# kxhit/SG_PR

Hardware: AMD Instinct MI355X
Metric: graph-pairs/sec (higher is better)
Workload: dtype f32 (2xf16-plane operands on the matrix cores, fp32 accumulate; fp32 vector math)

## Files before the change

sg_pr_amd/csrc/sgpr_score.hip:

```cpp
#include <math.h>

#include <string.h>

#include <type_traits>

#include "sgpr_internal.hpp"

namespace sgpr {

constexpr int F = kF3;
constexpr int T = kT;
constexpr int BN_ = kB;

__device__ __forceinline__ float ntn_neuron(const float* __restrict__ ntn_w, const float* __restrict__ ntn_wb,
                                            const float* __restrict__ bias, const float* __restrict__ e1,
                                            const float* __restrict__ e2, int lane) {
    const int t = lane & 15, q = lane >> 4;
    float v[8];
#pragma unroll
    for (int r = 0; r < 8; ++r) v[r] = 0.f;
    for (int i = 0; i < F; ++i) {
        const float a = e1[i];
        const float* wr = ntn_w + i * (F * T) + lane;
#pragma unroll
        for (int r = 0; r < 8; ++r) v[r] = fmaf(a, wr[64 * r], v[r]);
    }
    float s = 0.f;
#pragma unroll
    for (int r = 0; r < 8; ++r) s = fmaf(v[r], e2[q + 4 * r], s);
    for (int m = 0; m < 16; ++m) {
        const int mm = q * 16 + m;
        const float x = mm < F ? e1[mm] : e2[mm - F];
        s = fmaf(ntn_wb[t * 2 * F + mm], x, s);
    }
    s += __shfl_xor(s, 16);
    s += __shfl_xor(s, 32);
    return relu_keep_nan(s + bias[t]);
}

__global__ __launch_bounds__(256) void score_pairs_kernel(const DevWeights w, const float* __restrict__ p1,
                                                          const int32_t* __restrict__ i1,
                                                          const float* __restrict__ p2,
                                                          const int32_t* __restrict__ i2, int64_t P,
                                                          float* __restrict__ score) {
    const int lane = threadIdx.x & 63;
    const int64_t pair = (int64_t)blockIdx.x * 4 + (threadIdx.x >> 6);
    if (pair >= P) return;
    const int64_t r1 = i1 ? i1[pair] : pair;
    const int64_t r2 = i2 ? i2[pair] : pair;
    const int t = lane & 15;
    const float h = ntn_neuron(w.ntn_w, w.ntn_wb, w.ntn_bias, p1 + r1 * F, p2 + r2 * F, lane);
    float gacc = w.fc1_b[t];
    for (int tt = 0; tt < T; ++tt) gacc = fmaf(w.fc1_w[t * T + tt], __shfl(h, tt), gacc);
    float z = relu_keep_nan(gacc) * w.fc2_w[t];
    z += __shfl_xor(z, 1);
    z += __shfl_xor(z, 2);
    z += __shfl_xor(z, 4);
    z += __shfl_xor(z, 8);
    if (lane == 0) score[pair] = 1.f / (1.f + expf(-(z + w.fc2_b[0])));
}

__global__ __launch_bounds__(256) void ntn_kernel(const float* __restrict__ ntn_w, const float* __restrict__ ntn_wb,
                                                  const float* __restrict__ bias, const float* __restrict__ e1,
                                                  const float* __restrict__ e2, int64_t B, float* __restrict__ out) {
    const int lane = threadIdx.x & 63;
    const int64_t pair = (int64_t)blockIdx.x * 4 + (threadIdx.x >> 6);
    if (pair >= B) return;
    const float h = ntn_neuron(ntn_w, ntn_wb, bias, e1 + pair * F, e2 + pair * F, lane);
    if (lane < T) out[pair * T + lane] = h;
}

int launch_ntn(const float* w, const float* wb, const float* bias, const float* e1, const float* e2, int64_t B,
               float* out, hipStream_t stream) {
    if (B == 0) return SGPR_OK;
    const int64_t blocks = (B + 3) / 4;
    if (blocks > 0x7fffffffLL) {
        set_error("sgpr_ntn: too many pairs for one launch");
        return SGPR_E_INVALID;
    }
    hipLaunchKernelGGL(ntn_kernel, dim3((unsigned)blocks), dim3(256), 0, stream, w, wb, bias, e1, e2, B, out);
    hipError_t e = hipGetLastError();
    if (e != hipSuccess) return hip_fail(e, "ntn_kernel launch");
    return SGPR_OK;
}

int launch_score_pairs(const sgpr_handle* h, const float* p1, const int32_t* i1, const float* p2, const int32_t* i2,
                       int64_t P, float* score, hipStream_t stream) {
    if (P == 0) return SGPR_OK;
    const int64_t blocks = (P + 3) / 4;
    if (blocks > 0x7fffffffLL) {
        set_error("sgpr_score_pairs: too many pairs for one launch");
        return SGPR_E_INVALID;
    }
    hipLaunchKernelGGL(score_pairs_kernel, dim3((unsigned)blocks), dim3(256), 0, stream, h->w, p1, i1, p2, i2, P, score);
    hipError_t e = hipGetLastError();
    if (e != hipSuccess) return hip_fail(e, "score_pairs_kernel launch");
    return SGPR_OK;
}

constexpr int AP_RW = 4;
constexpr int AP_ROWS = 16;
constexpr int AP_SB = 64;
constexpr int AP_COLS = 256;
#ifndef SGPR_AP_OCC
#define SGPR_AP_OCC 4
#endif
constexpr int AP_MULTI_OCC = 3;
constexpr int AP_OCC = SGPR_AP_OCC;
#ifndef SGPR_AP_NI
#define SGPR_AP_NI 2
#endif
#ifndef SGPR_AP_CHAINS
#define SGPR_AP_CHAINS 1
#endif
#ifndef SGPR_AP_NT_STORE
#define SGPR_AP_NT_STORE 0
#endif
constexpr int AP_NI = SGPR_AP_NI;
constexpr float AP_F16_SAFE = 60000.f;

static inline int ap_prep_groups(int R, int M) {
    const int msb = (M + AP_SB - 1) / AP_SB * AP_SB;
    return ((R > msb ? R : msb) + 15) / 16;
}

size_t score_all_pairs_ws_bytes(int R, int M) {
    const size_t nsb = (size_t)(M + AP_SB - 1) / AP_SB;
    return (size_t)R * T * sizeof(float) + (size_t)2 * ap_prep_groups(R, M) * 4 * sizeof(float) +
           (size_t)R * 3 * 64 * 8 * sizeof(unsigned short) + nsb * 3 * 4 * 64 * 8 * sizeof(unsigned short);
}

struct ApOperands {
    float* ur;
    float* rng;
    unsigned short* Ab;
    unsigned short* Cb;
};
static ApOperands ap_operands(void* ws, int R, int nrng, int planes) {
    ApOperands o;
    o.ur = static_cast<float*>(ws);
    o.rng = o.ur + (size_t)R * T;
    o.Ab = reinterpret_cast<unsigned short*>(o.rng + (size_t)nrng * 4);
    o.Cb = o.Ab + (size_t)R * planes * 64 * 8;
    return o;
}

typedef float f32x4 __attribute__((ext_vector_type(4)));
typedef _Float16 f16x8 __attribute__((ext_vector_type(8)));
typedef _Float16 f16x2 __attribute__((ext_vector_type(2)));

__device__ __forceinline__ void split2_f16(float a, _Float16& h, _Float16& l) {
    h = (_Float16)a;
    l = (_Float16)(a - (float)h);
}

__device__ __forceinline__ void split3_bf16(float x, unsigned& hb, unsigned& mb, unsigned& lb) {
    hb = __float_as_uint(x);
    const float r1 = x - __uint_as_float(hb & 0xffff0000u);
    mb = __float_as_uint(r1);
    const float r2 = r1 - __uint_as_float(mb & 0xffff0000u);
    lb = __float_as_uint(r2);
}

__device__ __forceinline__ float range_max(float m, float x) { return fmaxf(m, x != x ? INFINITY : fabsf(x)); }

__device__ __forceinline__ float wave_max_f32(float v) {
    v = fmaxf(v, __shfl_xor(v, 1));
    v = fmaxf(v, __shfl_xor(v, 2));
    v = fmaxf(v, __shfl_xor(v, 4));
    v = fmaxf(v, __shfl_xor(v, 8));
    v = fmaxf(v, __shfl_xor(v, 16));
    return fmaxf(v, __shfl_xor(v, 32));
}

template <bool LIST, int NPL = 2>
__device__ __forceinline__ void ntn_prep_body(const DevWeights& w, const float* __restrict__ rows, int R,
                                              const float* __restrict__ cols, int M, unsigned short* __restrict__ Ab,
                                              float* __restrict__ ur, float* __restrict__ rng,
                                              unsigned short* __restrict__ Cb, const int block,
                                              const int32_t* __restrict__ row_ids = nullptr) {
    __shared__ float red[4][4];
    __shared__ __attribute__((aligned(16))) unsigned short stage[16 * NPL * 4 * 8 * 8];
    const int lane = threadIdx.x & 63, wave = threadIdx.x >> 6;
    const int l15 = lane & 15, lq = lane >> 4;
    const int g0 = (block >> 1) * 16, half = block & 1;
    float amax = 0.f, umax = 0.f, emax = 0.f, l1max = 0.f;
    if (g0 < R) {
        const int ga = min(g0 + l15, R - 1);
        const float* e = rows + (size_t)(LIST ? row_ids[ga] : ga) * F + 4 * lq;
        const float4 ea0 = *reinterpret_cast<const float4*>(e), ea1 = *reinterpret_cast<const float4*>(e + 16);
        float wv[4][8], wbv[4], l1r[4] = {0.f, 0.f, 0.f, 0.f};
#pragma unroll
        for (int q = 0; q < 4; ++q) {
            const int tile = half * 16 + wave * 4 + q;
            const int t = tile >> 1, j = (tile & 1) * 16 + l15;
            const float* wp = w.ntn_wt + ((size_t)(4 * lq) * T + t) * F + j;
#pragma unroll
            for (int s4 = 0; s4 < 4; ++s4) {
                wv[q][s4] = wp[s4 * T * F];
                wv[q][4 + s4] = wp[(16 + s4) * T * F];
            }
            wbv[q] = w.ntn_wb[t * 2 * F + F + j];
        }
#pragma unroll
        for (int q = 0; q < 4; ++q) {
            const int tile = half * 16 + wave * 4 + q;
            const int t = tile >> 1, j = (tile & 1) * 16 + l15;
            f32x4 acc = {0.f, 0.f, 0.f, 0.f};
            acc = __builtin_amdgcn_mfma_f32_16x16x4f32(ea0.x, wv[q][0], acc, 0, 0, 0);
            acc = __builtin_amdgcn_mfma_f32_16x16x4f32(ea0.y, wv[q][1], acc, 0, 0, 0);
            acc = __builtin_amdgcn_mfma_f32_16x16x4f32(ea0.z, wv[q][2], acc, 0, 0, 0);
            acc = __builtin_amdgcn_mfma_f32_16x16x4f32(ea0.w, wv[q][3], acc, 0, 0, 0);
            acc = __builtin_amdgcn_mfma_f32_16x16x4f32(ea1.x, wv[q][4], acc, 0, 0, 0);
            acc = __builtin_amdgcn_mfma_f32_16x16x4f32(ea1.y, wv[q][5], acc, 0, 0, 0);
            acc = __builtin_amdgcn_mfma_f32_16x16x4f32(ea1.z, wv[q][6], acc, 0, 0, 0);
            acc = __builtin_amdgcn_mfma_f32_16x16x4f32(ea1.w, wv[q][7], acc, 0, 0, 0);
            const float wbc = wbv[q];
            if ((q & 1) == 0) {
#pragma unroll
                for (int r = 0; r < 4; ++r) l1r[r] = 0.f;
            }
#pragma unroll
            for (int r = 0; r < 4; ++r) {
                const int g = g0 + 4 * lq + r;
                if (g < R) {
                    const float a = acc[r] + wbc;
                    amax = range_max(amax, a);
                    l1r[r] += fabsf(a);
                    unsigned short* dst = stage + (((4 * lq + r) * NPL * 4 + (j >> 3)) * 8 + (t & 7)) * 8 + (j & 7);
                    if constexpr (NPL == 3) {
                        unsigned hb, mb, lb;
                        split3_bf16(a, hb, mb, lb);
                        dst[0] = (unsigned short)(hb >> 16);
                        dst[4 * 8 * 8] = (unsigned short)(mb >> 16);
                        dst[2 * 4 * 8 * 8] = (unsigned short)(lb >> 16);
                    } else {
                        _Float16 h, l;
                        split2_f16(a, h, l);
                        dst[0] = __builtin_bit_cast(unsigned short, h);
                        dst[4 * 8 * 8] = __builtin_bit_cast(unsigned short, l);
                    }
                }
            }
            if (q & 1) {
#pragma unroll
                for (int r = 0; r < 4; ++r) {
                    float v = l1r[r];
                    v += __shfl_xor(v, 1);
                    v += __shfl_xor(v, 2);
                    v += __shfl_xor(v, 4);
                    v += __shfl_xor(v, 8);
                    l1max = fmaxf(l1max, v);
                }
            }
        }
    }
    if (g0 < R) {
        __syncthreads();
        for (int u = threadIdx.x; u < 16 * NPL * 4 * 8; u += 256) {
            const int tl = u & 7, jb = (u >> 3) & 3, pl = (u >> 5) % NPL, gi = (u >> 5) / NPL;
            if (g0 + gi < R)
                *reinterpret_cast<uint4*>(Ab + (((size_t)(g0 + gi) * NPL + pl) * 64 + jb * 16 + half * 8 + tl) * 8) =
                    *reinterpret_cast<const uint4*>(stage + (size_t)u * 8);
        }
    }
    for (int gi = half * 8 + wave * 2; gi < half * 8 + wave * 2 + 2; ++gi) {
        const int g = g0 + gi;
        if (g < R) {
            const float* e1 = rows + (size_t)(LIST ? row_ids[g] : g) * F;
            float s = 0.f;
            for (int m = 0; m < 8; ++m) s = fmaf(w.ntn_wb[l15 * 2 * F + lq * 8 + m], e1[lq * 8 + m], s);
            s += __shfl_xor(s, 16);
            s += __shfl_xor(s, 32);
            s += w.ntn_bias[l15];
            umax = range_max(umax, s);
            if (lq == 0) ur[(size_t)g * T + l15] = s;
        }
        const int msb = LIST ? M : (M + AP_SB - 1) / AP_SB * AP_SB;
        if (g < msb && lane < F) {
            const float x = g < M ? cols[(size_t)g * F + lane] : 0.f;
            emax = range_max(emax, x);
            _Float16 h, l;
            split2_f16(x, h, l);
            if (LIST) {
                unsigned short* dst = Cb + (size_t)g * (2 * F) + lane;
                dst[0] = __builtin_bit_cast(unsigned short, h);
                dst[F] = __builtin_bit_cast(unsigned short, l);
            } else {
                const int sb = g >> 6, cl = g & 63, c15 = cl >> 2, b = cl & 3, j = lane;
                unsigned short* dst = Cb + ((((size_t)sb * NPL) * 4 + b) * 64 + (j >> 3) * 16 + c15) * 8 + (j & 7);
                if constexpr (NPL == 3) {
                    unsigned hb, mb, lb;
                    split3_bf16(x, hb, mb, lb);
                    dst[0] = (unsigned short)(hb >> 16);
                    dst[4 * 64 * 8] = (unsigned short)(mb >> 16);
                    dst[2 * 4 * 64 * 8] = (unsigned short)(lb >> 16);
                } else {
                    dst[0] = __builtin_bit_cast(unsigned short, h);
                    dst[4 * 64 * 8] = __builtin_bit_cast(unsigned short, l);
                }
            }
        }
    }
    amax = wave_max_f32(amax);
    umax = wave_max_f32(umax);
    emax = wave_max_f32(emax);
    l1max = wave_max_f32(l1max);
    if (lane == 0) {
        red[wave][0] = amax;
        red[wave][1] = umax;
        red[wave][2] = emax;
        red[wave][3] = l1max;
    }
    __syncthreads();
    if (threadIdx.x < 4) {
        const int q = threadIdx.x;
        rng[(size_t)block * 4 + q] = fmaxf(fmaxf(red[0][q], red[1][q]), fmaxf(red[2][q], red[3][q]));
    }
}

__global__ __launch_bounds__(256) void ntn_prep_kernel(const DevWeights w, const float* __restrict__ rows, int R,
                                                       const float* __restrict__ cols, int M,
                                                       unsigned short* __restrict__ Ab, float* __restrict__ ur,
                                                       float* __restrict__ rng, unsigned short* __restrict__ Cb) {
    ntn_prep_body<false>(w, rows, R, cols, M, Ab, ur, rng, Cb, (int)blockIdx.x);
}

__global__ __launch_bounds__(256) void ntn_prep_wide_kernel(const DevWeights w, const float* __restrict__ rows, int R,
                                                            const float* __restrict__ cols, int M,
                                                            unsigned short* __restrict__ Ab, float* __restrict__ ur,
                                                            float* __restrict__ rng, unsigned short* __restrict__ Cb) {
    ntn_prep_body<false, 3>(w, rows, R, cols, M, Ab, ur, rng, Cb, (int)blockIdx.x);
}

constexpr int AP_MAX_JOBS = 8;
struct ApJob {
    const float* rows;
    const float* cols;
    float* score;
    int64_t ld;
    unsigned short* Ab;
    unsigned short* Cb;
    float* ur;
    float* rng;
    int R, M, nrng;
};
struct ApJobs {
    int n;
    int block0[AP_MAX_JOBS + 1];
    int item0[AP_MAX_JOBS + 1];
    ApJob job[AP_MAX_JOBS];
};

__global__ __launch_bounds__(256) void ntn_prep_multi_kernel(const DevWeights w, const ApJobs jobs) {
    int j = 0;
    while (j + 1 < jobs.n && (int)blockIdx.x >= jobs.block0[j + 1]) ++j;
    const ApJob& q = jobs.job[j];
    ntn_prep_body<false>(w, q.rows, q.R, q.cols, q.M, q.Ab, q.ur, q.rng, q.Cb, (int)blockIdx.x - jobs.block0[j]);
}

__device__ __forceinline__ f32x4 mfma_f16(f16x8 a, f16x8 b, f32x4 c) {
    return __builtin_amdgcn_mfma_f32_16x16x32_f16(a, b, c, 0, 0, 0);
}

__device__ __forceinline__ float swap32_add(float a, float b) {
    const auto r = __builtin_amdgcn_permlane32_swap(__float_as_uint(a), __float_as_uint(b), false, false);
    return __uint_as_float(r[0]) + __uint_as_float(r[1]);
}
__device__ __forceinline__ float swap16_add(float a, float b) {
    const auto r = __builtin_amdgcn_permlane16_swap(__float_as_uint(a), __float_as_uint(b), false, false);
    return __uint_as_float(r[0]) + __uint_as_float(r[1]);
}

__device__ __forceinline__ float relu(float x) { return __int_as_float(max(__float_as_int(x), 0)); }

typedef short i16x2 __attribute__((ext_vector_type(2)));
typedef unsigned u32x4 __attribute__((ext_vector_type(4)));
template <bool CL>
__device__ __forceinline__ f16x8 split_relu4(f32x4 h) {
    const unsigned h01 = __builtin_bit_cast(unsigned, __builtin_amdgcn_cvt_pkrtz(h[0], h[1]));
    const unsigned h23 = __builtin_bit_cast(unsigned, __builtin_amdgcn_cvt_pkrtz(h[2], h[3]));
    unsigned l01, l23;
    const i16x2 z = {0, 0};
    const unsigned a = __builtin_bit_cast(unsigned, __builtin_elementwise_max(__builtin_bit_cast(i16x2, h01), z));
    const unsigned b = __builtin_bit_cast(unsigned, __builtin_elementwise_max(__builtin_bit_cast(i16x2, h23), z));
    if constexpr (CL) {
        asm("v_fma_mixlo_f16 %0, %2, -1.0, %4 op_sel_hi:[1,0,0] clamp\n\t"
            "v_fma_mixlo_f16 %1, %3, -1.0, %6 op_sel_hi:[1,0,0] clamp\n\t"
            "v_fma_mixhi_f16 %0, %2, -1.0, %5 op_sel:[1,0,0] op_sel_hi:[1,0,0] clamp\n\t"
            "v_fma_mixhi_f16 %1, %3, -1.0, %7 op_sel:[1,0,0] op_sel_hi:[1,0,0] clamp"
            : "=&v"(l01), "=&v"(l23)
            : "v"(h01), "v"(h23), "v"(h[0]), "v"(h[1]), "v"(h[2]), "v"(h[3]));
        return __builtin_bit_cast(f16x8, u32x4{a, b, l01, l23});
    } else {
        asm("v_fma_mixlo_f16 %0, %2, -1.0, %4 op_sel_hi:[1,0,0]\n\t"
            "v_fma_mixlo_f16 %1, %3, -1.0, %6 op_sel_hi:[1,0,0]\n\t"
            "v_fma_mixhi_f16 %0, %2, -1.0, %5 op_sel:[1,0,0] op_sel_hi:[1,0,0]\n\t"
            "v_fma_mixhi_f16 %1, %3, -1.0, %7 op_sel:[1,0,0] op_sel_hi:[1,0,0]"
            : "=&v"(l01), "=&v"(l23)
            : "v"(h01), "v"(h23), "v"(h[0]), "v"(h[1]), "v"(h[2]), "v"(h[3]));
        const unsigned c = __builtin_bit_cast(unsigned, __builtin_elementwise_max(__builtin_bit_cast(i16x2, l01), z));
        const unsigned d = __builtin_bit_cast(unsigned, __builtin_elementwise_max(__builtin_bit_cast(i16x2, l23), z));
        return __builtin_bit_cast(f16x8, u32x4{a, b, c, d});
    }
}

__device__ __forceinline__ float slow_pair(const DevWeights& w, const float* __restrict__ e1, const float* __restrict__ e2) {
    const int lane = threadIdx.x & 63, t = lane & 15, q = lane >> 4;
    float s = 0.f;
#pragma unroll 1
    for (int j = 8 * q; j < 8 * q + 8; ++j) {
        float v = 0.f;
#pragma unroll 1
        for (int i = 0; i < F; ++i) v = fmaf(e1[i], w.ntn_w[i * (F * T) + j * T + t], v);
        s = fmaf(v, e2[j], s);
    }
#pragma unroll 1
    for (int m = 16 * q; m < 16 * q + 16; ++m) s = fmaf(w.ntn_wb[t * 2 * F + m], m < F ? e1[m] : e2[m - F], s);
    s += __shfl_xor(s, 16);
    s += __shfl_xor(s, 32);
    const float h = relu_keep_nan(s + w.ntn_bias[t]);
    float gacc = w.fc1_b[t];
#pragma unroll 1
    for (int tt = 0; tt < T; ++tt) gacc = fmaf(w.fc1_w[t * T + tt], __shfl(h, tt), gacc);
    float z = relu_keep_nan(gacc) * w.fc2_w[t];
    z += __shfl_xor(z, 1);
    z += __shfl_xor(z, 2);
    z += __shfl_xor(z, 4);
    z += __shfl_xor(z, 8);
    return 1.f / (1.f + expf(-(z + w.fc2_b[0])));
}

__device__ __forceinline__ void slow_tile(const DevWeights& w, const float* __restrict__ prow,
                                          const float* __restrict__ pcol, int r0, int r1, int c0, int c1,
                                          float* __restrict__ score, int64_t ld) {
    const int lane = threadIdx.x & 63;
#pragma unroll 1
    for (int r = r0; r < r1; ++r)
#pragma unroll 1
        for (int c = c0; c < c1; ++c) {
            const float sc = slow_pair(w, prow + (size_t)r * F, pcol + (size_t)c * F);
            if (lane == 0) score[(size_t)r * ld + c] = sc;
        }
}

struct ApConsts {
    f16x8 w1hi, w1lo;
    float4 b1v, side;
    float nb2, nl2e;
};

__device__ __forceinline__ ApConsts ap_consts(const DevWeights& w, int l15, int g) {
    ApConsts c;
    const float s = w.fc2_w[l15] * w.head_scale;
    float4 w1v = *reinterpret_cast<const float4*>(w.fc1_w + l15 * T + 4 * g);
    w1v = make_float4(s * w1v.x, s * w1v.y, s * w1v.z, s * w1v.w);
    const _Float16 wh0 = (_Float16)w1v.x, wh1 = (_Float16)w1v.y, wh2 = (_Float16)w1v.z, wh3 = (_Float16)w1v.w;
    const _Float16 z16 = (_Float16)0.f;
    c.w1hi = f16x8{wh0, wh1, wh2, wh3, wh0, wh1, wh2, wh3};
    c.w1lo = f16x8{(_Float16)(w1v.x - (float)wh0), (_Float16)(w1v.y - (float)wh1), (_Float16)(w1v.z - (float)wh2),
                        (_Float16)(w1v.w - (float)wh3), z16, z16, z16, z16};
    const float4 b1 = *reinterpret_cast<const float4*>(w.fc1_b + 4 * g);
    const float4 w2 = *reinterpret_cast<const float4*>(w.fc2_w + 4 * g);
    const float hs = w.head_scale;
    c.b1v = make_float4((w2.x * hs) * b1.x, (w2.y * hs) * b1.y, (w2.z * hs) * b1.z, (w2.w * hs) * b1.w);
    c.side = make_float4(w2.x < 0.f ? -INFINITY : INFINITY, w2.y < 0.f ? -INFINITY : INFINITY,
                         w2.z < 0.f ? -INFINITY : INFINITY, w2.w < 0.f ? -INFINITY : INFINITY);
    c.nb2 = -w.fc2_b[0] * 1.4426950408889634f;
    c.nl2e = w.head_nl2e;
    return c;
}

__device__ __forceinline__ void ap_range(const float* __restrict__ rng, int nrng, float& am, float& um, float& em, float& l1) {
    __shared__ float4 part[4];
    const float4 z = make_float4(0.f, 0.f, 0.f, 0.f);
    for (int i = threadIdx.x; i < nrng; i += 4 * 256) {
        const float4 v0 = *reinterpret_cast<const float4*>(rng + (size_t)i * 4);
        const float4 v1 = i + 256 < nrng ? *reinterpret_cast<const float4*>(rng + (size_t)(i + 256) * 4) : z;
        const float4 v2 = i + 512 < nrng ? *reinterpret_cast<const float4*>(rng + (size_t)(i + 512) * 4) : z;
        const float4 v3 = i + 768 < nrng ? *reinterpret_cast<const float4*>(rng + (size_t)(i + 768) * 4) : z;
        am = fmaxf(fmaxf(am, v0.x), fmaxf(fmaxf(v1.x, v2.x), v3.x));
        um = fmaxf(fmaxf(um, v0.y), fmaxf(fmaxf(v1.y, v2.y), v3.y));
        em = fmaxf(fmaxf(em, v0.z), fmaxf(fmaxf(v1.z, v2.z), v3.z));
        l1 = fmaxf(fmaxf(l1, v0.w), fmaxf(fmaxf(v1.w, v2.w), v3.w));
    }
    am = wave_max_f32(am);
    um = wave_max_f32(um);
    em = wave_max_f32(em);
    l1 = wave_max_f32(l1);
    if ((threadIdx.x & 63) == 0) part[threadIdx.x >> 6] = make_float4(am, um, em, l1);
    __syncthreads();
    const float4 p0 = part[0], p1 = part[1], p2 = part[2], p3 = part[3];
    am = fmaxf(fmaxf(p0.x, p1.x), fmaxf(p2.x, p3.x));
    um = fmaxf(fmaxf(p0.y, p1.y), fmaxf(p2.y, p3.y));
    em = fmaxf(fmaxf(p0.z, p1.z), fmaxf(p2.z, p3.z));
    l1 = fmaxf(fmaxf(p0.w, p1.w), fmaxf(p2.w, p3.w));
    __syncthreads();
}
__device__ __forceinline__ int ap_mode(float am, float um, float em, float l1) {
    if (!((am < AP_F16_SAFE) && (em < AP_F16_SAFE) && (um + 32.f * am * em < AP_F16_SAFE))) return 0;
    return (um + l1 * em < 1024.f) ? 2 : 1;
}

struct TopkArgs {
    const int32_t* row_self;
    int row0, window, causal, k, wg;
    float* val;
    int32_t* idx;
    float* pval;
    int32_t* pidx;
    int32_t* status;
};

constexpr int TK_EMPTY = 0x7fffffff;

__device__ __forceinline__ bool tk_beats(float av, int ac, float bv, int bc) { return av > bv || (av == bv && ac < bc); }


template <int K>
__device__ __forceinline__ void tk_merge(float& lv, int& lc, float cv, int cc, bool ok, float* sv, int* sc) {
    const int lane = threadIdx.x & 63, l15 = lane & 15, base = lane & 48;
    if (!ok) {
        cv = -INFINITY;
        cc = TK_EMPTY;
    }
    int rc = 0, rl = l15;
#pragma unroll
    for (int j = 0; j < 16; ++j) {
        const float ov = __shfl(cv, base + j);
        const int oc = __shfl(cc, base + j);
        rc += tk_beats(ov, oc, cv, cc) ? 1 : 0;
        rl += tk_beats(ov, oc, lv, lc) ? 1 : 0;
    }
#pragma unroll
    for (int j = 0; j < K; ++j) {
        const float ov = __shfl(lv, base + j);
        const int oc = __shfl(lc, base + j);
        rc += tk_beats(ov, oc, cv, cc) ? 1 : 0;
    }
    if (ok && rc < K) {
        sv[base + rc] = cv;
        sc[base + rc] = cc;
    }
    if (l15 < K && rl < K) {
        sv[base + rl] = lv;
        sc[base + rl] = lc;
    }
    __builtin_amdgcn_fence(__ATOMIC_RELEASE, "wavefront");
    __builtin_amdgcn_wave_barrier();
    __builtin_amdgcn_fence(__ATOMIC_ACQUIRE, "wavefront");
    if (l15 < K) {
        lv = sv[lane];
        lc = sc[lane];
    }
    __builtin_amdgcn_wave_barrier();
}

template <int K>
__device__ __forceinline__ void tk_push(const float (&sc)[4], int c0, int M, int ea, int eb, bool live, float& tv, int& tc,
                                        float& thv, int& thc, float* lsv, int* lsc) {
    if constexpr (K == 1) {
#pragma unroll
        for (int b = 0; b < 4; ++b) {
            const int c = c0 + b;
            const float v = sc[b];
            if (live && c < M && (c < ea || c > eb) && v == v && tk_beats(v, c, tv, tc)) {
                tv = v;
                tc = c;
            }
        }
    } else {
#pragma unroll
        for (int b = 0; b < 4; ++b) {
            const int c = c0 + b;
            const float v = sc[b];
            const bool q = live && c < M && (c < ea || c > eb) && v == v && tk_beats(v, c, thv, thc);
            if (__any(q)) {
                tk_merge<K>(tv, tc, v, c, q, lsv, lsc);
                const int src = (threadIdx.x & 48) + K - 1;
                thv = __shfl(tv, src);
                thc = __shfl(tc, src);
            }
        }
    }
}

template <int K, bool NEG = false>
__device__ __forceinline__ void tk_flush(const TopkArgs& a, int rg, int ncc, int it0, int it1, int r, int R, float tv, int tc) {
    const int lane = threadIdx.x & 63, l15 = lane & 15;
    if constexpr (K == 1) {
#pragma unroll
        for (int m = 1; m < 16; m <<= 1) {
            const float ov = __shfl_xor(tv, m);
            const int oc = __shfl_xor(tc, m);
            if (tk_beats(ov, oc, tv, tc)) {
                tv = ov;
                tc = oc;
            }
        }
    }
    if (r >= R || l15 >= a.k) return;
    if ((int64_t)rg * ncc >= it0 && (int64_t)(rg + 1) * ncc <= it1) {
        a.val[(size_t)r * a.k + l15] = NEG ? -tv : tv;
        a.idx[(size_t)r * a.k + l15] = tc == TK_EMPTY ? -1 : tc;
    } else {
        const int slot = rg == it0 / ncc ? 0 : 1;
        const size_t p = ((size_t)(a.wg * 2 + slot) * AP_ROWS + (r - rg * AP_ROWS)) * a.k + l15;
        a.pval[p] = tv;
        a.pidx[p] = tc;
    }
}

constexpr int TK_ABOVE = -1;

struct AboveArgs {
    const int32_t* row_self;
    int row0, window, causal, pass, wg;
// ... 1847 lines not shown
```

Before: 87.72 billion.

## Hoist prep-kernel loads ahead of MFMA and vectorize column split stores

```diff
diff --git a/sg_pr_amd/csrc/sgpr_score.hip b/sg_pr_amd/csrc/sgpr_score.hip
--- a/sg_pr_amd/csrc/sgpr_score.hip
+++ b/sg_pr_amd/csrc/sgpr_score.hip
@@ -181,15 +181,18 @@
                                               const int32_t* __restrict__ row_ids = nullptr) {
     __shared__ float red[4][4];
     __shared__ __attribute__((aligned(16))) unsigned short stage[16 * NPL * 4 * 8 * 8];
+    typedef float f32x4u __attribute__((ext_vector_type(4), aligned(4)));
     const int lane = threadIdx.x & 63, wave = threadIdx.x >> 6;
     const int l15 = lane & 15, lq = lane >> 4;
     const int g0 = (block >> 1) * 16, half = block & 1;
     float amax = 0.f, umax = 0.f, emax = 0.f, l1max = 0.f;
+    float4 ea0 = make_float4(0.f, 0.f, 0.f, 0.f), ea1 = ea0;
+    float wv[4][8], wbv[4], l1r[4] = {0.f, 0.f, 0.f, 0.f};
     if (g0 < R) {
         const int ga = min(g0 + l15, R - 1);
         const float* e = rows + (size_t)(LIST ? row_ids[ga] : ga) * F + 4 * lq;
-        const float4 ea0 = *reinterpret_cast<const float4*>(e), ea1 = *reinterpret_cast<const float4*>(e + 16);
-        float wv[4][8], wbv[4], l1r[4] = {0.f, 0.f, 0.f, 0.f};
+        ea0 = *reinterpret_cast<const float4*>(e);
+        ea1 = *reinterpret_cast<const float4*>(e + 16);
 #pragma unroll
         for (int q = 0; q < 4; ++q) {
             const int tile = half * 16 + wave * 4 + q;
@@ -202,6 +205,33 @@
             }
             wbv[q] = w.ntn_wb[t * 2 * F + F + j];
         }
+    }
+    const int gw = g0 + half * 8 + wave * 2;
+    f32x4 wu[2] = {}, eu[2][2] = {};
+    float ub = 0.f;
+    if (g0 + half * 8 < R) {
+        const float* wbp = w.ntn_wb + l15 * 2 * F + lq * 8;
+        wu[0] = *reinterpret_cast<const f32x4*>(wbp);
+        wu[1] = *reinterpret_cast<const f32x4*>(wbp + 4);
+        ub = w.ntn_bias[l15];
+#pragma unroll
+        for (int i = 0; i < 2; ++i) {
+            const int g = min(gw + i, R - 1);
+            const float* e1 = rows + (size_t)(LIST ? row_ids[g] : g) * F + lq * 8;
+            eu[i][0] = *reinterpret_cast<const f32x4*>(e1);
+            eu[i][1] = *reinterpret_cast<const f32x4*>(e1 + 4);
+        }
+    }
+    const int msb = LIST ? M : (M + AP_SB - 1) / AP_SB * AP_SB;
+    const int gc = gw + (lane >> 2), jq = lane & 3;
+    const bool ccol = lane < 8 && gc < msb;
+    f32x4u cv[2] = {f32x4u{0.f, 0.f, 0.f, 0.f}, f32x4u{0.f, 0.f, 0.f, 0.f}};
+    if (ccol && gc < M) {
+        const float* cp = cols + (size_t)gc * F + 8 * jq;
+        cv[0] = *reinterpret_cast<const f32x4u*>(cp);
+        cv[1] = *reinterpret_cast<const f32x4u*>(cp + 4);
+    }
+    if (g0 < R) {
 #pragma unroll
         for (int q = 0; q < 4; ++q) {
             const int tile = half * 16 + wave * 4 + q;
@@ -255,51 +285,54 @@
             }
         }
     }
-    if (g0 < R) {
-        __syncthreads();
-        for (int u = threadIdx.x; u < 16 * NPL * 4 * 8; u += 256) {
-            const int tl = u & 7, jb = (u >> 3) & 3, pl = (u >> 5) % NPL, gi = (u >> 5) / NPL;
-            if (g0 + gi < R)
-                *reinterpret_cast<uint4*>(Ab + (((size_t)(g0 + gi) * NPL + pl) * 64 + jb * 16 + half * 8 + tl) * 8) =
-                    *reinterpret_cast<const uint4*>(stage + (size_t)u * 8);
-        }
-    }
-    for (int gi = half * 8 + wave * 2; gi < half * 8 + wave * 2 + 2; ++gi) {
-        const int g = g0 + gi;
-        if (g < R) {
-            const float* e1 = rows + (size_t)(LIST ? row_ids[g] : g) * F;
+    asm volatile("" : "+v"(wu[0]), "+v"(wu[1]), "+v"(eu[0][0]), "+v"(eu[0][1]), "+v"(eu[1][0]), "+v"(eu[1][1]));
+    if (gw < R) {
+        const float wm[8] = {wu[0][0], wu[0][1], wu[0][2], wu[0][3], wu[1][0], wu[1][1], wu[1][2], wu[1][3]};
+#pragma unroll
+        for (int i = 0; i < 2; ++i) {
+            const float em[8] = {eu[i][0][0], eu[i][0][1], eu[i][0][2], eu[i][0][3], eu[i][1][0], eu[i][1][1], eu[i][1][2], eu[i][1][3]};
             float s = 0.f;
-            for (int m = 0; m < 8; ++m) s = fmaf(w.ntn_wb[l15 * 2 * F + lq * 8 + m], e1[lq * 8 + m], s);
+#pragma unroll
+            for (int m = 0; m < 8; ++m) s = fmaf(wm[m], em[m], s);
             s += __shfl_xor(s, 16);
             s += __shfl_xor(s, 32);
-            s += w.ntn_bias[l15];
-            umax = range_max(umax, s);
-            if (lq == 0) ur[(size_t)g * T + l15] = s;
-        }
-        const int msb = LIST ? M : (M + AP_SB - 1) / AP_SB * AP_SB;
-        if (g < msb && lane < F) {
-            const float x = g < M ? cols[(size_t)g * F + lane] : 0.f;
-            emax = range_max(emax, x);
-            _Float16 h, l;
-            split2_f16(x, h, l);
-            if (LIST) {
-                unsigned short* dst = Cb + (size_t)g * (2 * F) + lane;
-                dst[0] = __builtin_bit_cast(unsigned short, h);
-                dst[F] = __builtin_bit_cast(unsigned short, l);
+            s += ub;
+            if (gw + i < R) {
+                umax = range_max(umax, s);
+                if (lq == 0) ur[(size_t)(gw + i) * T + l15] = s;
+            }
+        }
+    }
+    if (ccol) {
+        const float x[8] = {cv[0][0], cv[0][1], cv[0][2], cv[0][3], cv[1][0], cv[1][1], cv[1][2], cv[1][3]};
+        unsigned short pl[NPL][8];
+#pragma unroll
+        for (int m = 0; m < 8; ++m) {
+            emax = range_max(emax, x[m]);
+            if constexpr (NPL == 3) {
+                unsigned hb, mb, lb;
+                split3_bf16(x[m], hb, mb, lb);
+                pl[0][m] = (unsigned short)(hb >> 16);
+                pl[1][m] = (unsigned short)(mb >> 16);
+                pl[2][m] = (unsigned short)(lb >> 16);
             } else {
-                const int sb = g >> 6, cl = g & 63, c15 = cl >> 2, b = cl & 3, j = lane;
-                unsigned short* dst = Cb + ((((size_t)sb * NPL) * 4 + b) * 64 + (j >> 3) * 16 + c15) * 8 + (j & 7);
-                if constexpr (NPL == 3) {
-                    unsigned hb, mb, lb;
-                    split3_bf16(x, hb, mb, lb);
-                    dst[0] = (unsigned short)(hb >> 16);
-                    dst[4 * 64 * 8] = (unsigned short)(mb >> 16);
-                    dst[2 * 4 * 64 * 8] = (unsigned short)(lb >> 16);
-                } else {
-                    dst[0] = __builtin_bit_cast(unsigned short, h);
-                    dst[4 * 64 * 8] = __builtin_bit_cast(unsigned short, l);
-                }
-            }
+                _Float16 h, l;
+                split2_f16(x[m], h, l);
+                pl[0][m] = __builtin_bit_cast(unsigned short, h);
+                pl[1][m] = __builtin_bit_cast(unsigned short, l);
+            }
+        }
+        const int sb = gc >> 6, cl = gc & 63, c15 = cl >> 2, b = cl & 3;
+        unsigned short* dst = LIST ? Cb + (size_t)gc * (2 * F) + 8 * jq
+                                   : Cb + ((((size_t)sb * NPL) * 4 + b) * 64 + jq * 16 + c15) * 8;
+#pragma unroll
+        for (int p = 0; p < NPL; ++p) {
+            uint4 u;
+            u.x = pl[p][0] | ((unsigned)pl[p][1] << 16);
+            u.y = pl[p][2] | ((unsigned)pl[p][3] << 16);
+            u.z = pl[p][4] | ((unsigned)pl[p][5] << 16);
+            u.w = pl[p][6] | ((unsigned)pl[p][7] << 16);
+            *reinterpret_cast<uint4*>(dst + (size_t)p * (LIST ? F : 4 * 64 * 8)) = u;
         }
     }
     amax = wave_max_f32(amax);
@@ -313,6 +346,14 @@
         red[wave][3] = l1max;
     }
     __syncthreads();
+    if (g0 < R) {
+        for (int u = threadIdx.x; u < 16 * NPL * 4 * 8; u += 256) {
+            const int tl = u & 7, jb = (u >> 3) & 3, pl = (u >> 5) % NPL, gi = (u >> 5) / NPL;
+            if (g0 + gi < R)
+                *reinterpret_cast<uint4*>(Ab + (((size_t)(g0 + gi) * NPL + pl) * 64 + jb * 16 + half * 8 + tl) * 8) =
+                    *reinterpret_cast<const uint4*>(stage + (size_t)u * 8);
+        }
+    }
     if (threadIdx.x < 4) {
         const int q = threadIdx.x;
         rng[(size_t)block * 4 + q] = fmaxf(fmaxf(red[0][q], red[1][q]), fmaxf(red[2][q], red[3][q]));
```

Measured after the change: 87.78 billion (median of 4 runs). About the same (+0.1%).
